# tancredeguillou/diner

Measured on AMD Instinct MI355X. Metric: rendered rays/sec (512x512, 4 src views, 128 samples/ray), higher is better.
Workload: dtype f32 (GEMM operands split into fp16 hi+lo, 3 fp16 MFMAs per product, fp32 accumulate)

## Files before the change

### diner_amd/_lib.py

```python
from __future__ import annotations

import ctypes as C
from pathlib import Path

import torch

LIB_PATH = Path(__file__).resolve().parent / "lib" / "libdiner_hip.so"
_FP = C.c_void_p

N_BLOCKS, COMBINE = 5, 3
ABI_VERSION = 3
PRECISIONS = {"fp32": 0, "f16x3": 1}
ROUNDINGS = {"save_image": 0, "video": 1}
BG_RULES = {"none": 0, "below_half": 1, "below_one": 2}
RESIZE_MODES = {"bilinear_aa": 1, "bilinear": 2, "bicubic_u8": 3}
ACT_NONE, ACT_RELU, ACT_SOFTPLUS = 0, 1, 2


class DinerScene(C.Structure):
    _fields_ = [("SB", C.c_int32), ("NV", C.c_int32), ("H", C.c_int32), ("W", C.c_int32),
                ("h", C.c_int32), ("w", C.c_int32), ("C", C.c_int32), ("num_freqs", C.c_int32),
                ("image_w", C.c_float), ("image_h", C.c_float), ("feature_padding", C.c_float),
                ("freq_factor", C.c_float),
                ("poses", _FP), ("focal", _FP), ("c", _FP), ("maps", _FP), ("latent", _FP), ("linz_maps", _FP)]
# ... 67 lines not shown
    "diner_gen_rays": (C.c_int, [_P, _P, _P, _P, _I32, _I32, _I32, _P, _P]),
    "diner_gen_rays_backward_workspace_floats": (_I64, [_I32, _I32, _I32]),
    "diner_gen_rays_backward": (C.c_int, [_P, _P, _P, _I32, _I32, _I32, _P, _P, _P, _P, _P, _P]),
    "diner_depth2normal": (C.c_int, [_P, _P, _I32, _I32, _I32, _P, _P]),
    "diner_pack_maps": (C.c_int, [_P, _P, _P, _I64, _I32, _I32, _P, _P]),
    "diner_pack_maps_from_depth": (C.c_int, [_P, _P, _P, _I64, _I32, _I32, _P, _P]),
    "diner_pack_latent": (C.c_int, [_P, _I64, _I32, _I32, _I32, _P, _P]),
    "diner_mlp_packed_floats": (_I64, []),
    "diner_pack_mlp": (C.c_int, [C.POINTER(DinerMlpRaw), _P, _P]),
    "diner_pack_linz_maps": (C.c_int, [_P, _I64, _I32, _I32, _P, _P, _P]),
    "diner_sample_coarse": (C.c_int, [_P, _I64, _I32, _P, _U64, _P, _P]),
    "diner_sample_depthguided": (C.c_int, [C.POINTER(DinerScene), _P, _I64, C.POINTER(DinerSamplerCfg),
                                           _P, _P, _P, _P, _U64, _P, _P, _P, _P]),
    "diner_fill_up_uniform_samples": (C.c_int, [_P, _P, _I64, _I32, _P, _U64, _P, _P]),
    "diner_render_points_scratch_floats": (_I64, [_I64, _I32, _I32]),
    "diner_render_points": (C.c_int, [C.POINTER(DinerScene), _P, _P, _P, _I64, _I32, _I32, _P, _P, _P]),
    "diner_composite": (C.c_int, [_P, _P, _P, _I64, _I32, _I32, _P, _P, _P, _P, _P]),
    "diner_decode_depth_u16": (C.c_int, [_P, _P, _P, _I64, _I32, _I32, _I32, C.c_float, C.c_float, C.c_float, C.c_float, C.c_float,
                                         _P, _P, _P, _P]),
    "diner_train_gemm": (C.c_int, [_P, _P, _P, _P, _P, _I64, _I32, _I32, _I64, _I64, _I64, _I64, _I64, _I64, _I32, _I32, _I32, _I32, _I64,
                                   _I32, _P, _P, _I32, _I32, _P]),
    "diner_train_amax": (C.c_int, [_P, _I64, _P, _P]),
    "diner_train_colsum_amax": (C.c_int, [_P, _I64, _I32, _I64, _P, _P, _P]),
    "diner_train_split_panel": (C.c_int, [_P, _I32, _I64, _I32, _I32, _P, _P, _P]),
    "diner_train_pack_core": (C.c_int, [_P, _I64, _I32, _I32, _P, _P]),
    "diner_train_gemm_core": (C.c_int, [_P, _I64, _P, _P, _P, _I64, _P, _I64, _P, _I64, _I64, _I32, _P, _I32, _I32, _P, _P, _P]),
    "diner_train_gemm_panel": (C.c_int, [_P, _I64, _P, _P, _P, _P, _I64, _P, _I64, _P, _I64, _I64, _I32, _I32, _P, _I32, _I32, _P]),
    "diner_train_colsum": (C.c_int, [_P, _I64, _I32, _I64, _P, _P]),
    "diner_train_point_inputs": (C.c_int, [C.POINTER(DinerScene), _P, _I32, _P, _P, _I64, _I32, _I32, _P, _P, _P, _P]),
    "diner_train_bilinear_scatter": (C.c_int, [_P, _P, _I64, _I32, _I32, _I32, _I32, _I32, _P, _P]),
# ... 146 lines not shown
        if not LIB_PATH.exists():
            raise ImportError(
                f"{LIB_PATH} is missing: the MI355X render path has no CPU or PyTorch fallback. "
                "Build it with `make -C diner_amd/csrc` (hipcc --offload-arch=gfx950).")
        l = C.CDLL(str(LIB_PATH))
        for name, (res, args) in SYMBOLS.items():
            fn = getattr(l, name)
            fn.restype, fn.argtypes = res, args
        if l.diner_version() != ABI_VERSION:
            raise ImportError(f"{LIB_PATH} has ABI version {l.diner_version()}, this binding needs {ABI_VERSION}: rebuild it "
                              "(`make -C diner_amd/csrc`)")
        _lib = l
    return _lib


def check(rc: int, what: str) -> None:
    if rc != 0:
        msg = lib().diner_last_error().decode(errors="replace")
        if rc == -1:
            raise ValueError(f"{what}: {msg}")
        if rc == -3:
            raise NotImplementedError(f"{what}: {msg}")
        raise DinerHipError(f"{what}: {msg} (rc={rc})")
```

### diner_amd/csrc/api.hip

```cpp
#include <stdarg.h>
#include <stdio.h>

#include <atomic>

#include "common.hpp"

namespace diner {

static thread_local char g_err[512] = "";

void set_error(const char *fmt, ...)
{
    va_list ap;
    va_start(ap, fmt);
    vsnprintf(g_err, sizeof(g_err), fmt, ap);
    va_end(ap);
}

int check_launch(const char *what)
{
    const hipError_t e = hipGetLastError();
    if (e != hipSuccess) {
        set_error("%s: %s", what, hipGetErrorString(e));
        return DINER_E_LAUNCH;
// ... 77 lines not shown
int launch_decode_depth(const unsigned short *, const unsigned short *, const unsigned short *, int64_t, int, int, int, float, float, float,
                        float, float, float *, float *, float *, hipStream_t);
int launch_linz_maps(const float *, int64_t, const float *, float *, hipStream_t);
int launch_linz_maps_ring(const float *, int64_t, int, int, const float *, float *, hipStream_t);
int launch_sampler(const DinerScene &, const float *, const DinerTargetCam *, float *, int64_t, const DinerSamplerCfg &, const float *,
                   const float *, const float *, const float *, uint64_t, float *, float *, float *, hipStream_t);
int launch_sampler_points(const DinerScene &, const float *, const float *, const float *, int64_t, const DinerSamplerCfg &, const float *,
                          const float *, uint64_t, float *, float *, float *, hipStream_t);
int launch_sample_coarse(const float *, int64_t, int, const float *, uint64_t, float *, hipStream_t);
int launch_fill_up(const float *, const float *, int64_t, int, const float *, uint64_t, float *, hipStream_t);
int launch_points_mlp(const DinerScene &, const DinerLatentIndex &, const float *, const float *, const float *, int64_t, int, float *, hipStream_t);
int64_t mlp_f16_packed_floats();
int launch_pack_mlp_f16(const DinerMlpRaw &, float *, hipStream_t);
int launch_points_mlp_f16(const DinerScene &, const DinerLatentIndex &, const float *, const float *, const float *, int64_t, int, float *, float *, hipStream_t);
int64_t points_mlp_f16_scratch_floats(int64_t SB, int NV);
namespace gen {
int check_shape(const DinerMlpShape &);
int64_t packed_floats(const DinerMlpShape &);
int launch_pack_mlp(const DinerMlpShape &, const DinerMlpGenRaw &, float *, hipStream_t);
int launch_points_mlp(const DinerScene &, const DinerLatentIndex &, const DinerMlpShape &, const float *, const float *, const float *, int64_t, int, float *, hipStream_t,
                      int bicubic_pad = -1);
int launch_points_mlp_lz(const DinerScene &, const DinerLatentIndex &, const DinerMlpShape &, const float *, const float *, const float *, int64_t, int, float *,
                         hipStream_t, int bicubic_pad, const float *lzmaps);
int64_t linz_maps_floats(const DinerMlpShape &, int64_t texels);
int launch_linz_maps(const DinerMlpShape &, const float *, int64_t, const float *, float *, hipStream_t);
int launch_points_mlp_novel(const DinerScene &, const DinerLatentIndex &, const DinerNovelGen &, const DinerMlpShape &, const float *, const float *,
                            const float *, const float *, int64_t, float *, hipStream_t);
int launch_points_mlp_novel_pe(const DinerScene &, const DinerLatentIndex &, const DinerNovelGen &, const DinerNovelPe &, const DinerMlpShape &,
                               const float *, const float *, const float *, const float *, const float *, int64_t, float *, hipStream_t);
int launch_novel_pe_map(const float *, int64_t, int, const float *, float *, hipStream_t);
// ... 233 lines not shown
    if (N < 0 || h <= 0 || w <= 0) return bad("linz_maps_floats: bad size");
    const int r = (index && index->padding == DINER_INDEX_PAD_ZEROS) ? 1 : 0;
    return 3 * N * (int64_t)(h + 2 * r) * (w + 2 * r) * DINER_D_LATENT;
}

int diner_pack_linz_maps_ix(const float *latent_packed, int64_t N, int32_t h, int32_t w, const float *mlp_packed,
                            const DinerLatentIndex *index, float *out, void *stream)
{
    int rc;
    if ((rc = check_index(index, "pack_linz_maps_ix"))) return rc;
    if (!index || index->padding != DINER_INDEX_PAD_ZEROS) return diner_pack_linz_maps(latent_packed, N, h, w, mlp_packed, out, stream);
    if (!latent_packed || !mlp_packed || !out) return bad("pack_linz_maps_ix: NULL pointer");
    if (N < 0 || h <= 0 || w <= 0) return bad("pack_linz_maps_ix: bad size");
    return launch_linz_maps_ring(latent_packed, N, h, w, mlp_packed, out, (hipStream_t)stream);
}

int64_t diner_render_points_scratch_floats(int64_t SB, int32_t NV, int32_t precision)
{
    return precision == DINER_PRECISION_F16X3 ? points_mlp_f16_scratch_floats(SB, NV) : 0;
}

int diner_render_points(const DinerScene *scene, const float *mlp_packed, const float *rays, const float *z,
                        int64_t NR, int32_t K, int32_t precision, float *scratch, float *rgbsigma_out, void *stream)
{
    return diner_render_points_ix(scene, nullptr, mlp_packed, rays, z, NR, K, precision, scratch, rgbsigma_out, stream);
}

int diner_render_points_ix(const DinerScene *scene, const DinerLatentIndex *index, const float *mlp_packed, const float *rays,
                           const float *z, int64_t NR, int32_t K, int32_t precision, float *scratch, float *rgbsigma_out, void *stream)
{
// ... 827 lines not shown
```

### diner_amd/csrc/common.hpp

```cpp
#pragma once
#include <hip/hip_runtime.h>
#include <stdint.h>

#include "../../include/diner_hip.h"

#define DINER_WAVE 64
#define DINER_SIGMA_PAD 100

namespace diner {

void set_error(const char *fmt, ...);
int check_launch(const char *what);

int device_cus();
enum LdsSlot { LDS_SLOT_F16_LINZ = 0, LDS_SLOT_F16_LATENT = 2, LDS_SLOT_F16_TRACE = 4, LDS_SLOT_TRAIN_CORE0 = 6, LDS_SLOT_DW512 = 10,
               LDS_SLOT_F16_GIX = 12, LDS_SLOT_COUNT = 16 };
int ensure_dynamic_lds(const void *kernel, int bytes, int slot);

struct View {
    float r[9];
    float t[3];
    float fx, fy, cx, cy;
};

__device__ __forceinline__ View load_view(const DinerScene &s, int sb, int v)
{
    View o;
    const float *P = s.poses + ((int64_t)sb * s.NV + v) * 16;
#pragma unroll
    for (int i = 0; i < 3; ++i) {
        o.r[i * 3 + 0] = P[i * 4 + 0];
// ... 315 lines not shown
```

### diner_amd/csrc/points_mlp_f16.hip

```cpp
#include <stdio.h>
#include <stdlib.h>

#include <type_traits>

#include "common.hpp"

namespace diner {

typedef float f32x16 __attribute__((ext_vector_type(16)));
typedef float f32x4 __attribute__((ext_vector_type(4)));
typedef _Float16 h8 __attribute__((ext_vector_type(8)));
typedef _Float16 h4 __attribute__((ext_vector_type(4)));
typedef unsigned u32x2 __attribute__((ext_vector_type(2)));

namespace f16x3 {

#include "f16_core16.inc"
#ifdef DINER_F16_DIAG
#include "f16_core16_trace.inc"
#endif
static_assert(F16_SHAPE == 16, "this kernel's glue is written for the 16x16x32 accumulator layout");

constexpr int TILE_P = 64;
constexpr int NWAVES = 8;
// ... 33 lines not shown
    int nkb, in_dim;
    if (i < OFF_LIN_Z) { w = raw.lin_in_w; rel = i; nkb = NKB_IN; in_dim = DINER_D_IN; }
    else if (i < OFF_FC0) { const int b = (int)((i - OFF_LIN_Z) / W_FULL); w = raw.lin_z_w[b]; rel = (i - OFF_LIN_Z) % W_FULL; nkb = NKB_FULL; in_dim = HID; }
    else if (i < OFF_FC1) { const int b = (int)((i - OFF_FC0) / W_FULL); w = raw.fc0_w[b]; rel = (i - OFF_FC0) % W_FULL; nkb = NKB_FULL; in_dim = HID; }
    else { const int b = (int)((i - OFF_FC1) / W_FULL); w = raw.fc1_w[b]; rel = (i - OFF_FC1) % W_FULL; nkb = NKB_FULL; in_dim = HID; }
    const int j = (int)(rel & 7), lane = (int)((rel >> 3) & 63), part = (int)((rel >> 9) & 1), tf2 = (int)((rel >> 10) & 1), hs = (int)((rel >> 11) & 1);
    const int64_t blk = rel >> 12;
    const int nks = nkb / 2, ks = (int)(blk % nks), wv = (int)(blk / nks);
    const int n = wv * 64 + 16 * (2 * hs + tf2) + (lane & 15), k = ks * 32 + 8 * (lane >> 4) + j;
    const float v = k < in_dim ? w[(int64_t)n * in_dim + k] : 0.0f;
    const _Float16 hi = (_Float16)v;
    outw[i] = part == 0 ? hi : (_Float16)(v - (float)hi);
}
#endif

template <int I, int N, class F> __device__ __forceinline__ void sfor(F &&f)
{
    if constexpr (I < N) {
        f(std::integral_constant<int, I>{});
        sfor<I + 1, N>(f);
    }
}
template <int N> __device__ __forceinline__ float acc_read()
{
    float v;
    asm volatile("v_mov_b32 %0, v%c1" : "=v"(v) : "n"(N));
    return v;
}
template <int N> __device__ __forceinline__ void acc_write(float v)
{
// ... 4 lines not shown
    asm volatile("v_add_f32 v%c0, v%c0, %1" ::"n"(N), "v"(v));
}
template <int N> __device__ __forceinline__ void acc_load4(const float *p)
{
    asm volatile("global_load_dwordx4 v[%c0:%c1], %2, off" ::"n"(N), "n"(N + 3), "v"(p) : "memory");
}
typedef __attribute__((address_space(1))) f32x4 g_f32x4;
typedef __attribute__((address_space(1))) unsigned g_u32;
typedef __attribute__((address_space(3))) volatile unsigned lds_vu32;
__device__ __forceinline__ f32x4 gload4(const float *p) { return *(const g_f32x4 *)p; }
__device__ __forceinline__ void gstore4(float *p, f32x4 v)
{
    asm volatile("global_store_dwordx4 %0, %1, off\n\ts_nop 3" ::"v"(p), "v"(v) : "memory");
}
template <int BASE, int TF, int TP, int I> constexpr int areg() { return BASE + 4 * (4 * TF + TP) + I; }

__device__ __forceinline__ void split(float s, _Float16 &hi, _Float16 &lo)
{
    hi = (_Float16)s;
    lo = (_Float16)(s - (float)hi);
}

constexpr int IMG_BYTES = 128 * 1024;
struct Tap {
    unsigned o00, o01, o10, o11;
    float nw, ne, sw, se;
};
constexpr int LDS_TAPS = IMG_BYTES;
constexpr int LDS_BIAS = LDS_TAPS + TILE_P * 32;
constexpr int LDS_FLAG = LDS_BIAS + BIAS_FLOATS * 4;
// ... 93 lines not shown
                     "v_pk_add_f32 v[%c[a2]:%c[a3]], v[%c[a2]:%c[a3]], v[%c[d2]:%c[d3]]\n\t"
                     "global_store_dwordx4 %[px], v[%c[x00]:%c[x03]], off\n\t"
                     "global_store_dwordx4 %[pn], v[%c[a0]:%c[a3]], off\n\t"
                     "s_nop 3"
                     ::[a0] "n"(n0), [a1] "n"(n0 + 1), [a2] "n"(n0 + 2), [a3] "n"(n0 + 3), [d0] "n"(n3), [d1] "n"(n3 + 1), [d2] "n"(n3 + 2), [d3] "n"(n3 + 3),
                       [x00] "n"(x0), [x01] "n"(x0 + 1), [x02] "n"(x0 + 2), [x03] "n"(x0 + 3), [x30] "n"(x3), [x31] "n"(x3 + 1), [x32] "n"(x3 + 2), [x33] "n"(x3 + 3),
                       [px] "v"(px), [pn] "v"(pn)
                     : "memory");
}

constexpr int SLAB_FLOATS = TILE_P * HID;
constexpr int PACE_EVERY = 4;
constexpr int TRACE_EVENTS = 512;
constexpr int SYNC_WORDS = 256;

template <bool LINZ, bool TRACE, bool VIT, class... IX>
__global__ __launch_bounds__(NWAVES * 64) __attribute__((amdgpu_num_vgpr(F16_VGPR_CAP / 2)))    void points_mlp_f16_kernel(
    DinerScene s, const float *__restrict__ Wp, const float *__restrict__ rays, const float *__restrict__ zsamp, int64_t NR, int K,
    int64_t tiles, float *__restrict__ scratch, float *__restrict__ rgbsigma, unsigned long long *__restrict__ dbg, IX... ix)
{
    constexpr bool GIX = sizeof...(IX) == 2;
    const int ixv[] = {ix..., 0, 0};
    const int ix_interp = GIX ? ixv[0] : 0, ix_padding = GIX ? ixv[1] : 0;
    int ev = 0;
    bool trace_on = false;
#define EV(ID)                                                                                   \
    if (TRACE && trace_on) {                                                                     \
        const unsigned long long t_ = __builtin_amdgcn_s_memtime();                              \
        if (lane == 0 && ev < TRACE_EVENTS) dbg[(wave * TRACE_EVENTS + ev) * 2] = t_, dbg[(wave * TRACE_EVENTS + ev) * 2 + 1] = ID; \
        ++ev;                                                                                    \
    }
#ifndef DINER_F16_DIAG
#define LAYER(FN, ...) FN(__VA_ARGS__)
#else
#define LAYER(FN, ...)                                                                           \
    do {                                                                                         \
        if constexpr (TRACE) {                                                                   \
// ... 30 lines not shown
        asm volatile("" : "+s"(b));
        (void)tn;
        return b + (uint64_t)(off_halfs * 2);
    };
    auto win = [&](int tn) -> uint64_t {
        uint64_t b = wbase_in;
        asm volatile("" : "+s"(b));
        (void)tn;
        return b;
    };
    const int ring = (GIX && LINZ && ix_padding == DINER_INDEX_PAD_ZEROS) ? 1 : 0;
    const int mw = s.w + 2 * ring, mh = s.h + 2 * ring;
    auto gmap = [&](int b, int v) -> uint64_t {
        uint64_t g = (uint64_t)(uintptr_t)s.linz_maps;
        asm volatile("" : "+s"(g));
        return g + (uint64_t)((((int64_t)b * s.SB + sb) * s.NV + v) * mh * mw) * (HID * 4);
    };
    GatherRegs greg;
    {
        const unsigned pl = lane >> 4, quad = lane & 15, stage = (unsigned)(uintptr_t)img + wave * 16384;
        greg.tbase = (unsigned)(uintptr_t)taps + pl * 32;
        greg.qb = wave * 256 + quad * 16;
#pragma unroll
        for (int k = 0; k < 4; ++k) greg.sw[k] = stage + pl * 256 + (((quad ^ pl) ^ (4 * k)) << 4);
        greg.rb = stage + c16 * 256;
        greg.hp = q ^ c16;
    }
    const unsigned loff = lane * 16;
    const unsigned ab0 = (unsigned)(uintptr_t)img + q * 2048 + c16 * 16;
    float *slab0 = scratch + SYNC_WORDS + ((int64_t)blockIdx.y * gridDim.x + blockIdx.x) * (int64_t)(2 * SLAB_FLOATS) + lane * 4;
    float *xs = slab0 + wave * (64 * 64);
// ... 29 lines not shown
                __hip_atomic_fetch_add(pace, 1u, __ATOMIC_RELAXED, __HIP_MEMORY_SCOPE_AGENT);
                const unsigned int want = (unsigned int)(round / PACE_EVERY + 1) * group;
                int spin = 0;
                for (; spin < 4000; ++spin) {
                    if (__hip_atomic_load(pace, __ATOMIC_RELAXED, __HIP_MEMORY_SCOPE_AGENT) >= want) break;
                    __builtin_amdgcn_s_sleep(8);
                }
                pace_flag[0] = spin < 4000;
            }
            __builtin_amdgcn_s_waitcnt(0xC07F);
            __builtin_amdgcn_s_barrier();
            pace_on = pace_flag[0] != 0;
        }
        trace_on = TRACE && blockIdx.x == 0 && blockIdx.y == 0 && round == 2;
        EV(1)
        int64_t p = tile * TILE_P + lane;
        if (p > P - 1) p = P - 1;
        const int64_t ray = p / K;
        const float *rp = rays + ((int64_t)sb * NR + ray) * 8;
        const float zz = zsamp[(int64_t)sb * P + p];
        const float dwx0 = rp[3], dwy0 = rp[4], dwz0 = rp[5];
        const float wx0 = rp[0] + zz * dwx0, wy0 = rp[1] + zz * dwy0, wz0 = rp[2] + zz * dwz0;
        float dwx = dwx0, dwy = dwy0, dwz = dwz0, wx = wx0, wy = wy0, wz = wz0;
        const int NG = VIT ? s.NV / 4 : 1;
        const int nph = VIT ? 4 * NG : s.NV;

#pragma unroll 1
        for (int ph = 0; ph < nph; ++ph) {
            const int v = VIT ? 4 * (ph % NG) : ph;
            const int sub = VIT ? ph / NG : 0;
            {
                const int tpv = VIT ? lane >> 4 : 0;
                if (VIT) {
                    const int src = 16 * sub + (lane & 15);
                    wx = __shfl(wx0, src, 64); wy = __shfl(wy0, src, 64); wz = __shfl(wz0, src, 64);
                    dwx = __shfl(dwx0, src, 64); dwy = __shfl(dwy0, src, 64); dwz = __shfl(dwz0, src, 64);
                }
                const View vw = load_view(s, sb, v + tpv);
                float px, py, pz, u, w;
                project(vw, s.image_w, s.image_h, wx, wy, wz, px, py, pz, u, w);
                float dcx, dcy, dcz;
                rotate(vw, dwx, dwy, dwz, dcx, dcy, dcz);
                const int row8 = (wave + 3) & 7;
                float delta = 0.0f;
                if ((unsigned)(row8 - 5) < 2u) {
                    const float4 *tex = (const float4 *)s.maps + ((int64_t)sb * s.NV + v + tpv) * s.H * s.W * 2;
                    const int ddx = safe_idx(__builtin_rintf(clipf(unnorm(u, (float)s.W / 2.0f), (float)(s.W - 1))), s.W);
                    const int ddy = safe_idx(__builtin_rintf(clipf(unnorm(w, (float)s.H / 2.0f), (float)(s.H - 1))), s.H);
                    delta = tex[((int64_t)ddy * s.W + ddx) * 2].w - pz;
                }
                const float half_pi = 1.5707963267948966f;
#pragma unroll 1
                for (int e8 = 0; e8 < 8; ++e8) {
                    const int e = row8 * 8 + e8;
                    _Float16 *cell = (_Float16 *)(img + row8 * 2048 + lane * 16);
                    const bool pe3 = e >= 3 && e < 39, pe1 = e >= 43 && e < 55;
                    const int j = pe3 ? (e - 3) / 3 : e - 43, i = pe3 ? (e - 3) % 3 : e < 3 ? e : e - 39;
                    const float comp = i == 0 ? px : i == 1 ? py : pz, dcomp = i == 0 ? dcx : i == 1 ? dcy : dcz;
                    const float src = pe1 ? delta : comp;
                    float sn = 0.0f;
                    if (pe3 || pe1) sn = pe_sin(__builtin_fmaf(src, s.freq_factor * (float)(1 << ((j >> 1) & 7)), (j & 1) ? half_pi : 0.0f));
// ... 20 lines not shown
            }
            if (LINZ) {
                EV(10) LAYER(layer_x_in0, win(0), win(1), wfull(OFF_FC0, 0), wfull(OFF_FC0, 1), loff, ab0, (++sy.lay, sy)); EV(11)
            } else {
                acc_bias<X, false>(bias, wave, q);
                EV(10) LAYER(layer_x_in, win(0), win(1), wfull(OFF_LIN_Z, 0), wfull(OFF_LIN_Z, 1), loff, ab0, (++sy.lay, sy)); EV(11)
            }

#pragma unroll 1
            for (int b = 0; b < DINER_COMBINE_LAYER; ++b) {
                if (LINZ) {
                    if (b == 0) gather_finish<false>(gmap(b, v), greg);
                    else gather_finish<true>(gmap(b, v), greg);
                    EV(60)
                } else {
                    const f32x4 *lat = (const f32x4 *)s.latent + ((int64_t)sb * s.NV + v) * s.h * s.w * (HID / 4);
                    const int half = wave >> 2, ur = half * 32 + c;
#pragma unroll 1
                    for (int r0 = 0; r0 < 16; r0 += 2) {
                        const int row = (wave & 3) * 16 + r0 + h;
                        const Tap t = taps[row];
                        h8 vh, vl;
#pragma unroll
                        for (int hf = 0; hf < 2; ++hf) {
                            const int q = 2 * ur + hf;
                            const f32x4 a = lat[t.o00 + q], bq = lat[t.o01 + q], cq = lat[t.o10 + q], d = lat[t.o11 + q];
#pragma unroll
                            for (int i = 0; i < 4; ++i) {
                                const float o = __builtin_fmaf(d[i], t.se, __builtin_fmaf(cq[i], t.sw, __builtin_fmaf(bq[i], t.ne, a[i] * t.nw)));
                                _Float16 hi, lo;
                                split(o * ACT_SCALE, hi, lo);
// ... 17 lines not shown
                    const bool to_in = b == DINER_COMBINE_LAYER - 1 && ph < nph - 1;
                    const uint64_t n0 = to_in ? win(0) : wfull(OFF_FC1 + b * W_FULL, 0), n1 = to_in ? win(1) : wfull(OFF_FC1 + b * W_FULL, 1);
                    EV(20) LAYER(layer_net_full, wfull(OFF_FC0 + b * W_FULL, 0), wfull(OFF_FC0 + b * W_FULL, 1), n0, n1, loff, ab0, (++sy.lay, sy)); EV(21)
                }
                if (b < DINER_COMBINE_LAYER - 1) {
                    store_relu<NET>(img, wave, c16, q);
                    EV(51)
                    if (!LINZ) acc_bias<X, true>(bias + 512 * (9 + b), wave, q);
                    EV(52)
                    const int64_t nxt = LINZ ? OFF_FC0 + (b + 1) * W_FULL : OFF_LIN_Z + (b + 1) * W_FULL;
                    if (LINZ) gather_issue(gmap(b + 1, v), greg);
                    EV(53)
                    EV(30) LAYER(layer_x_full, wfull(OFF_FC1 + b * W_FULL, 0), wfull(OFF_FC1 + b * W_FULL, 1), wfull(nxt, 0), wfull(nxt, 1), loff, ab0, (++sy.lay, sy)); EV(31)
                }
            }
            if (!VIT && v < s.NV - 1) {
                float *sl = xs;
                asm volatile("" : "+v"(sl));
                sfor<0, 4>([&](auto B4) {
                    f32x4 ax[4], an[4];
                    if (v > 0)
                        sfor<0, 4>([&](auto Q) { constexpr int Gq = 4 * B4 + Q; ax[Q.value] = gload4(sl + Gq * 256); an[Q.value] = gload4(sl + SLAB_FLOATS + Gq * 256); });
                    sfor<0, 4>([&](auto Q) {
                        constexpr int Gq = 4 * B4 + Q;
                        f32x4 vx, vn;
                        sfor<0, 4>([&](auto J) {
                            vx[J.value] = acc_read<X + 4 * Gq + J>();
                            const float n = acc_read<NET + 4 * Gq + J>();
                            vn[J.value] = n < 0.0f ? 0.0f : n;
                        });
                        if (v > 0) { vx = ax[Q.value] + vx; vn = an[Q.value] + vn; }
                        gstore4(sl + Gq * 256, vx);
                        gstore4(sl + SLAB_FLOATS + Gq * 256, vn);
                    });
                });
            }
            if (VIT) {
                const bool last = ph == nph - 1;
                float *sl = slab0 + sub * (2 * 8192) + wave * 1024;
                asm volatile("" : "+v"(sl));
                const bool part = v > 0;
                if (part) {
                    f32x4 px = gload4(sl), pn = gload4(sl + 8192);
                    sfor<0, 4>([&](auto TF) {
                        constexpr int tf = TF.value;
                        f32x4 qx = px, qn = pn;
                        if (tf < 3) { px = gload4(sl + (tf + 1) * 256); pn = gload4(sl + 8192 + (tf + 1) * 256); }
                        f32x4 sx, sn;
                        sfor<0, 4>([&](auto J) {
                            constexpr int j = J.value;
                            float ax = acc_read<areg<X, tf, 0, j>()>();
                            float n0 = acc_read<areg<NET, tf, 0, j>()>();
                            float an = n0 < 0.0f ? 0.0f : n0;
                            ax = qx[j] + ax; an = qn[j] + an;
                            sfor<1, 4>([&](auto TP) {
                                ax = ax + acc_read<areg<X, tf, TP.value, j>()>();
                                const float n = acc_read<areg<NET, tf, TP.value, j>()>();
// ... 5 lines not shown
                        if (last) {
                            sfor<0, 4>([&](auto J) { acc_write<areg<X, tf, 3, J.value>()>(sx[J.value]); acc_write<areg<NET, tf, 3, J.value>()>(sn[J.value]); });
                        } else {
                            gstore4(sl + tf * 256, sx);
                            gstore4(sl + 8192 + tf * 256, sn);
                        }
                    });
                }
                else if (last) sfor<0, 4>([&](auto TF) { vit_sum_tile<TF.value, true>(nullptr, nullptr); });
                else sfor<0, 4>([&](auto TF) { vit_sum_tile<TF.value, false>(sl + TF.value * 256, sl + 8192 + TF.value * 256); });
            }
        }
#pragma unroll 1
        for (int b = DINER_COMBINE_LAYER - 1; b < DINER_N_BLOCKS; ++b) {
            if (b == DINER_COMBINE_LAYER - 1) {
                const float nv = (float)s.NV;
                const bool pow2 = (s.NV & (s.NV - 1)) == 0;
                const float rnv = 1.0f / nv;
                const float *b1 = bias + 512 * (9 + DINER_COMBINE_LAYER - 1);
                const float *sl = xs;
                asm volatile("" : "+v"(sl));
                if (VIT) {
                    const float *sp = slab0 + wave * 1024;
                    asm volatile("" : "+v"(sp));
                    sfor<0, 12>([&](auto I) {
                        constexpr int sb3 = I.value / 4, tf = I.value % 4;
                        acc_load4<areg<X, tf, sb3, 0>()>(sp + sb3 * (2 * 8192) + tf * 256);
                        acc_load4<areg<NET, tf, sb3, 0>()>(sp + sb3 * (2 * 8192) + 8192 + tf * 256);
                    });
                    asm volatile("s_waitcnt vmcnt(0)" ::: "memory");
                }
                auto mean_step = [&](auto POW2) {
                sfor<0, 4>([&](auto B4) {
                    f32x4 ax[4], an[4];
                    if (!VIT && s.NV > 1)
                        sfor<0, 4>([&](auto Q) { constexpr int Gq = 4 * B4 + Q; ax[Q.value] = gload4(sl + Gq * 256); an[Q.value] = gload4(sl + SLAB_FLOATS + Gq * 256); });
                    sfor<0, 4>([&](auto Q) {
                        constexpr int Gq = 4 * B4 + Q, tf = Gq / 4, tp = Gq % 4;
                        f32x4 sx, sn;
                        sfor<0, 4>([&](auto J) {
                            sx[J.value] = acc_read<X + 4 * Gq + J>();
                            const float n = acc_read<NET + 4 * Gq + J>();
                            sn[J.value] = n < 0.0f ? 0.0f : n;
                        });
                        if (!VIT && s.NV > 1) { sx = ax[Q.value] + sx; sn = an[Q.value] + sn; }
                        const f32x4 bb = *(const f32x4 *)(b1 + wave * 64 + tf * 16 + 4 * q);
                        h4 vh, vl;
                        sfor<0, 4>([&](auto J) {
                            acc_write<X + 4 * Gq + J>((POW2.value ? sx[J.value] * rnv : sx[J.value] / nv) + bb[J.value]);
                            _Float16 hi, lo;
                            split(POW2.value ? sn[J.value] * rnv : sn[J.value] / nv, hi, lo);
                            vh[J.value] = hi;
                            vl[J.value] = lo;
                        });
                        char *pc = img + (wave * 8 + tf * 2 + (q >> 1)) * 2048 + (tp * 16 + c16) * 16 + 8 * (q & 1);
                        *(h4 *)pc = vh;
                        *(h4 *)(pc + 1024) = vl;
                    });
                });
                };
                if (pow2) mean_step(std::true_type{});
                else mean_step(std::false_type{});
            } else {
                store_relu<X>(img, wave, c16, q);
                acc_bias<NET, false>(bias + 512 * (4 + b), wave, q);
                EV(20) LAYER(layer_net_full, wfull(OFF_FC0 + b * W_FULL, 0), wfull(OFF_FC0 + b * W_FULL, 1), wfull(OFF_FC1 + b * W_FULL, 0),
                               wfull(OFF_FC1 + b * W_FULL, 1), loff, ab0, (++sy.lay, sy)); EV(21)
                store_relu<NET>(img, wave, c16, q);
                acc_bias<X, true>(bias + 512 * (9 + b), wave, q);
            }
            const bool last = b == DINER_N_BLOCKS - 1;
            const uint64_t n0 = last ? win(0) : wfull(OFF_FC0 + (b + 1) * W_FULL, 0), n1 = last ? win(1) : wfull(OFF_FC0 + (b + 1) * W_FULL, 1);
            EV(30) LAYER(layer_x_full, wfull(OFF_FC1 + b * W_FULL, 0), wfull(OFF_FC1 + b * W_FULL, 1), n0, n1, loff, ab0, (++sy.lay, sy)); EV(31)
        }
        {
            float part[4][4] = {};
            sfor<0, 4>([&](auto TF) {
                constexpr int tf = TF.value;
                const int f = wave * 64 + tf * 16 + 4 * q;
                f32x4 wo[4];
#pragma unroll
                for (int o = 0; o < 4; ++o) wo[o] = *(const f32x4 *)(Wout + o * 512 + f);
                sfor<0, 16>([&](auto PJ) {
                    constexpr int tp = PJ / 4, j = PJ % 4;
                    const float xv = acc_read<areg<X, tf, tp, j>()>();
                    const float a = xv < 0.0f ? 0.0f : xv;
#pragma unroll
                    for (int o = 0; o < 4; ++o) part[tp][o] = __builtin_fmaf(a, wo[o][j], part[tp][o]);
                });
            });
            f32x4 mine;
#pragma unroll
            for (int o = 0; o < 4; ++o) {
                float sel = 0.0f;
#pragma unroll
                for (int tp = 0; tp < 4; ++tp) {
                    float t = part[tp][o];
// ... 11 lines not shown
                flow_signal(sy.ctr + 16, sy.one);
                if (wave >= 4) head_ok = flow_wait(sy.ctr + 16, 8 * tiles_done);
            } else {
                __builtin_amdgcn_s_waitcnt(0xC07F);
                __builtin_amdgcn_s_barrier();
            }
            EV(41)
            if (wave >= 4) {
                const int t = tid - 256, pt = t >> 2, o = t & 3;
                float sum = 0.0f;
#pragma unroll
                for (int w8 = 0; w8 < 8; ++w8) sum += *(const float *)(img + head_slot(w8) + pt * 16 + o * 4);
                if (F16_FLOW && *(lds_vu32 *)(lds + LDS_CTR + F16_POISON_OFF) != 0) head_ok = false;
                if (!head_ok) sum = __builtin_nanf("");
                const float val = (sum + bias[14 * 512 + o]) * (1.0f / ACT_SCALE);
                const int64_t pp = tile * TILE_P + pt;
                if (pp < P) rgbsigma[((int64_t)sb * P + pp) * 4 + o] = o < 3 ? 1.0f / (1.0f + expf(-val)) : (val < 0.0f ? 0.0f : val);
            }
            EV(42)
        }
    }
#undef EV
#undef LAYER
    if (!F16_FLOW && wave < 4) __builtin_amdgcn_s_barrier();
    asm volatile("s_waitcnt vmcnt(0)" ::: "memory");
}

}

#ifndef DINER_F16_KERNEL_ONLY
int64_t mlp_f16_packed_floats() { return f16x3::PACKED_FLOATS; }

int launch_pack_mlp_f16(const DinerMlpRaw &raw, float *out, hipStream_t st)
{
    using namespace f16x3;
    hipLaunchKernelGGL(pack_kernel, dim3((unsigned)((W_HALFS + 255) / 256)), dim3(256), 0, st, raw, (_Float16 *)out,
                       out + W_HALFS / 2);
    return check_launch("f16x3::pack_kernel");
}

const void *points_mlp_f16_gix_kernel(bool linz, bool vit);

static bool getenv_no_vit()
{
    static const bool off = getenv("DINER_F16_NO_VIT") != nullptr;
    return off;
}

static int f16_grid_limit() { return device_cus(); }

int64_t points_mlp_f16_scratch_floats(int64_t SB, int NV)
{
    return f16x3::SYNC_WORDS + (NV > 1 ? (int64_t)f16_grid_limit() * SB * 2 * f16x3::SLAB_FLOATS : 0);
}

int launch_points_mlp_f16(const DinerScene &s, const DinerLatentIndex &ix, const float *mlp_packed, const float *rays, const float *z,
                          int64_t NR, int K, float *scratch, float *rgbsigma, hipStream_t st)
{
    using namespace f16x3;
    const int64_t P = NR * (int64_t)K;
    if (P == 0 || s.SB == 0) return DINER_OK;
    if (s.C != DINER_D_LATENT) { set_error("render_points: latent channels C=%d unsupported (need %d)", s.C, DINER_D_LATENT); return DINER_E_UNSUPPORTED; }
    if (s.num_freqs != 6) { set_error("render_points: num_freqs=%d unsupported (need 6)", s.num_freqs); return DINER_E_UNSUPPORTED; }
    if (!scratch) { set_error("render_points(f16x3): scratch is NULL"); return DINER_E_INVALID; }
    if (hipMemsetAsync(scratch, 0, SYNC_WORDS * sizeof(float), st) != hipSuccess) return check_launch("memset(pacing counters)");
    const int64_t tiles = (P + TILE_P - 1) / TILE_P;
    const int64_t grid = tiles < f16_grid_limit() ? tiles : f16_grid_limit();
    const bool vit = s.NV % 4 == 0 && !getenv_no_vit();
    const bool gix = ix.interp != DINER_INDEX_BILINEAR || ix.padding != DINER_INDEX_PAD_BORDER;
    const void *fn = gix ? points_mlp_f16_gix_kernel(s.linz_maps != nullptr, vit)
                         : (s.linz_maps ? (vit ? (const void *)points_mlp_f16_kernel<true, false, true> : (const void *)points_mlp_f16_kernel<true, false, false>)
                                        : (vit ? (const void *)points_mlp_f16_kernel<false, false, true> : (const void *)points_mlp_f16_kernel<false, false, false>));
    if (const int rc = ensure_dynamic_lds(fn, LDS_BYTES, (s.linz_maps ? LDS_SLOT_F16_LINZ : LDS_SLOT_F16_LATENT) + (vit ? 1 : 0) + (gix ? LDS_SLOT_F16_GIX : 0)))
        return rc;
    const int ii = ix.interp, ip = ix.padding;
#ifdef DINER_F16_DIAG
    static const bool trace = getenv("DINER_F16_TRACE") != nullptr;
    if (trace && s.linz_maps && gix) {
        set_error("render_points(f16x3): DINER_F16_TRACE serves the bilinear / border lookup only (index interp=%d padding=%d)", ii, ip);
        return DINER_E_UNSUPPORTED;
    }
    if (trace && s.linz_maps) {
        static unsigned long long *dbg = nullptr;
        const size_t nb = NWAVES * TRACE_EVENTS * 2 * sizeof(unsigned long long);
        if (!dbg && hipMalloc(&dbg, nb) != hipSuccess) return DINER_E_LAUNCH;
        (void)hipMemsetAsync(dbg, 0, nb, st);
        const void *tfn = vit ? (const void *)points_mlp_f16_kernel<true, true, true> : (const void *)points_mlp_f16_kernel<true, true, false>;
        if (const int rc = ensure_dynamic_lds(tfn, LDS_BYTES, LDS_SLOT_F16_TRACE + (vit ? 1 : 0))) return rc;
        void *targs[] = {(void *)&s, (void *)&mlp_packed, (void *)&rays, (void *)&z, (void *)&NR, (void *)&K, (void *)&tiles, (void *)&scratch, (void *)&rgbsigma, (void *)&dbg};
        if (hipLaunchKernel(tfn, dim3((unsigned)grid, (unsigned)s.SB), dim3(NWAVES * 64), targs, LDS_BYTES, st) != hipSuccess) return check_launch("points_mlp_f16_kernel<trace>(launch)");
        static unsigned long long h[NWAVES * TRACE_EVENTS * 2];
        (void)hipStreamSynchronize(st);
        (void)hipMemcpy(h, dbg, nb, hipMemcpyDeviceToHost);
        for (int w = 0; w < NWAVES; ++w) {
            fprintf(stderr, "[f16 trace] wave%d:", w);
            for (int e = 0; e < TRACE_EVENTS && h[(w * TRACE_EVENTS + e) * 2 + 1]; ++e)
                fprintf(stderr, " %llu:%llu", h[(w * TRACE_EVENTS + e) * 2 + 1], h[(w * TRACE_EVENTS + e) * 2] - h[0]);
            fprintf(stderr, "\n");
        }
        return check_launch("points_mlp_f16_kernel<trace>");
    }
#endif
    unsigned long long *nodbg = nullptr;
    void *kargs[] = {(void *)&s, (void *)&mlp_packed, (void *)&rays, (void *)&z, (void *)&NR, (void *)&K, (void *)&tiles, (void *)&scratch, (void *)&rgbsigma, (void *)&nodbg, (void *)&ii, (void *)&ip};
    if (hipLaunchKernel(fn, dim3((unsigned)grid, (unsigned)s.SB), dim3(NWAVES * 64), kargs, LDS_BYTES, st) != hipSuccess)
        return check_launch("points_mlp_f16_kernel(launch)");
    return check_launch("points_mlp_f16_kernel");
}
#endif

}
```

### include/diner_hip.h

```cpp
#ifndef DINER_HIP_H
#define DINER_HIP_H

#include <stdint.h>

#ifdef __cplusplus
extern "C" {
#endif

#define DINER_OK 0
#define DINER_E_INVALID (-1)
#define DINER_E_LAUNCH (-2)
#define DINER_E_UNSUPPORTED (-3)

#define DINER_D_LATENT 512
#define DINER_D_HIDDEN 512
#define DINER_D_IN 55
#define DINER_N_BLOCKS 5
#define DINER_COMBINE_LAYER 3
#define DINER_MAP_TEXEL 8

#define DINER_PRECISION_FP32 0
#define DINER_PRECISION_F16X3 1

typedef struct DinerScene {
// ... 111 lines not shown
int diner_sample_coarse(const float *rays, int64_t N, int32_t NC, const float *u_coarse, uint64_t seed,
                        float *z_out, void *stream);
int diner_fill_up_uniform_samples(const float *rays, const float *z_in, int64_t N, int32_t K,
                                  const float *u_fill, uint64_t seed, float *z_out, void *stream);

int diner_sample_depthguided(const DinerScene *scene, const float *rays, int64_t NR,
                             const DinerSamplerCfg *cfg, const float *u_coarse,
                             const float *n_gauss, const float *u_fill, const float *z_cand,
                             uint64_t seed, float *z_out, float *z_dg_out, float *lik_out,
                             void *stream);

int64_t diner_render_points_scratch_floats(int64_t SB, int32_t NV, int32_t precision);
int diner_render_points(const DinerScene *scene, const float *mlp_packed, const float *rays,
                        const float *z, int64_t NR, int32_t K, int32_t precision, float *scratch,
                        float *rgbsigma_out, void *stream);
int diner_render_points_ix(const DinerScene *scene, const DinerLatentIndex *index, const float *mlp_packed, const float *rays,
                           const float *z, int64_t NR, int32_t K, int32_t precision, float *scratch, float *rgbsigma_out,
                           void *stream);

#define DINER_STATUS_NONFINITE 1u
int diner_composite(const float *rays, const float *z, const float *rgbsigma, int64_t N, int32_t K,
                    int32_t white_bkgd, float *rgb_out, float *depth_out, float *weights_out,
                    uint32_t *status, void *stream);

int64_t diner_render_workspace_floats(int64_t SB, int64_t NR, int32_t K, int32_t NV, int32_t precision);
int diner_render(const DinerScene *scene, const float *mlp_packed, const float *rays, int64_t NR,
                 const DinerSamplerCfg *cfg, int32_t white_bkgd, int32_t precision, const float *u_coarse,
                 const float *n_gauss, const float *u_fill, uint64_t seed, float *workspace,
                 float *rgb_out, float *depth_out, float *weights_out, uint32_t *status, void *stream);
int diner_render_ix(const DinerScene *scene, const DinerLatentIndex *index, const float *mlp_packed, const float *rays, int64_t NR,
// ... 295 lines not shown
```

Measured before the change: 265,200.

## Add compile-time four-view specialization of f16 points MLP kernel with 32-bit indexing

Adds a template specialization of the f16x3 points MLP kernel where the view count is a compile-time constant (4). With a fixed count the compiler can fold view-dependent address arithmetic, pick the power-of-two mean path statically and skip the partial-sum global reload in the views-in-tile reduction. It also switches to 32-bit index arithmetic when sizes allow and loads output weights through scalar registers. The change adds a separate kernel instantiation and LDS slot, plus a debug query that reports which variant last ran. It only applies when NV==4 with linz maps and the default index mode.

```diff
diff --git a/diner_amd/_lib.py b/diner_amd/_lib.py
--- a/diner_amd/_lib.py
+++ b/diner_amd/_lib.py
@@ -105,6 +105,7 @@
                                            _P, _P, _P, _P, _U64, _P, _P, _P, _P]),
     "diner_fill_up_uniform_samples": (C.c_int, [_P, _P, _I64, _I32, _P, _U64, _P, _P]),
     "diner_render_points_scratch_floats": (_I64, [_I64, _I32, _I32]),
+    "diner_points_mlp_f16_last_kernel": (_I32, []),
     "diner_render_points": (C.c_int, [C.POINTER(DinerScene), _P, _P, _P, _I64, _I32, _I32, _P, _P, _P]),
     "diner_composite": (C.c_int, [_P, _P, _P, _I64, _I32, _I32, _P, _P, _P, _P, _P]),
     "diner_decode_depth_u16": (C.c_int, [_P, _P, _P, _I64, _I32, _I32, _I32, C.c_float, C.c_float, C.c_float, C.c_float, C.c_float,
@@ -281,6 +282,14 @@
     return _lib
 
 
+F16_KERNEL_BITS = {"linz": 1, "vit": 2, "gix": 4, "nv4": 8, "idx32": 16}
+
+
+def f16_last_kernel():
+    code = int(lib().diner_points_mlp_f16_last_kernel())
+    return None if code < 0 else frozenset(k for k, b in F16_KERNEL_BITS.items() if code & b)
+
+
 def check(rc: int, what: str) -> None:
     if rc != 0:
         msg = lib().diner_last_error().decode(errors="replace")
diff --git a/diner_amd/csrc/api.hip b/diner_amd/csrc/api.hip
--- a/diner_amd/csrc/api.hip
+++ b/diner_amd/csrc/api.hip
@@ -115,6 +115,7 @@
 int launch_pack_mlp_f16(const DinerMlpRaw &, float *, hipStream_t);
 int launch_points_mlp_f16(const DinerScene &, const DinerLatentIndex &, const float *, const float *, const float *, int64_t, int, float *, float *, hipStream_t);
 int64_t points_mlp_f16_scratch_floats(int64_t SB, int NV);
+int points_mlp_f16_last_kernel();
 namespace gen {
 int check_shape(const DinerMlpShape &);
 int64_t packed_floats(const DinerMlpShape &);
@@ -378,6 +379,8 @@
     if (N < 0 || h <= 0 || w <= 0) return bad("pack_linz_maps_ix: bad size");
     return launch_linz_maps_ring(latent_packed, N, h, w, mlp_packed, out, (hipStream_t)stream);
 }
+
+int32_t diner_points_mlp_f16_last_kernel(void) { return points_mlp_f16_last_kernel(); }
 
 int64_t diner_render_points_scratch_floats(int64_t SB, int32_t NV, int32_t precision)
 {
diff --git a/diner_amd/csrc/common.hpp b/diner_amd/csrc/common.hpp
--- a/diner_amd/csrc/common.hpp
+++ b/diner_amd/csrc/common.hpp
@@ -14,7 +14,7 @@
 
 int device_cus();
 enum LdsSlot { LDS_SLOT_F16_LINZ = 0, LDS_SLOT_F16_LATENT = 2, LDS_SLOT_F16_TRACE = 4, LDS_SLOT_TRAIN_CORE0 = 6, LDS_SLOT_DW512 = 10,
-               LDS_SLOT_F16_GIX = 12, LDS_SLOT_COUNT = 16 };
+               LDS_SLOT_F16_GIX = 12, LDS_SLOT_F16_NV4 = 16, LDS_SLOT_COUNT = 18 };
 int ensure_dynamic_lds(const void *kernel, int bytes, int slot);
 
 struct View {
diff --git a/diner_amd/csrc/points_mlp_f16.hip b/diner_amd/csrc/points_mlp_f16.hip
--- a/diner_amd/csrc/points_mlp_f16.hip
+++ b/diner_amd/csrc/points_mlp_f16.hip
@@ -1,6 +1,7 @@
 #include <stdio.h>
 #include <stdlib.h>
 
+#include <atomic>
 #include <type_traits>
 
 #include "common.hpp"
@@ -71,6 +72,12 @@
 }
 #endif
 
+template <int N> struct NvViews { int idx32; };
+template <class... IX> struct nvc_of { static constexpr int value = 0; };
+template <int N> struct nvc_of<NvViews<N>> { static constexpr int value = N; };
+__device__ __forceinline__ int ix_word(int v) { return v; }
+template <int N> __device__ __forceinline__ int ix_word(NvViews<N> v) { return v.idx32; }
+
 template <int I, int N, class F> __device__ __forceinline__ void sfor(F &&f)
 {
     if constexpr (I < N) {
@@ -105,6 +112,22 @@
     asm volatile("global_store_dwordx4 %0, %1, off\n\ts_nop 3" ::"v"(p), "v"(v) : "memory");
 }
 template <int BASE, int TF, int TP, int I> constexpr int areg() { return BASE + 4 * (4 * TF + TP) + I; }
+
+__device__ __forceinline__ View load_view_at(const DinerScene &s, int64_t i)
+{
+    View o;
+    const float *P = s.poses + i * 16;
+#pragma unroll
+    for (int r = 0; r < 3; ++r) {
+        o.r[r * 3 + 0] = P[r * 4 + 0];
+        o.r[r * 3 + 1] = P[r * 4 + 1];
+        o.r[r * 3 + 2] = P[r * 4 + 2];
+        o.t[r] = P[r * 4 + 3];
+    }
+    const float *f = s.focal + i * 2, *c = s.c + i * 2;
+    o.fx = f[0]; o.fy = f[1]; o.cx = c[0]; o.cy = c[1];
+    return o;
+}
 
 __device__ __forceinline__ void split(float s, _Float16 &hi, _Float16 &lo)
 {
@@ -228,13 +251,17 @@
 constexpr int TRACE_EVENTS = 512;
 constexpr int SYNC_WORDS = 256;
 
+#define DINER_SNV (NVC ? NVC : s.NV)
 template <bool LINZ, bool TRACE, bool VIT, class... IX>
 __global__ __launch_bounds__(NWAVES * 64) __attribute__((amdgpu_num_vgpr(F16_VGPR_CAP / 2)))    void points_mlp_f16_kernel(
     DinerScene s, const float *__restrict__ Wp, const float *__restrict__ rays, const float *__restrict__ zsamp, int64_t NR, int K,
     int64_t tiles, float *__restrict__ scratch, float *__restrict__ rgbsigma, unsigned long long *__restrict__ dbg, IX... ix)
 {
+    constexpr int NVC = nvc_of<IX...>::value;
+    static_assert(NVC == 0 || (VIT && NVC % 4 == 0), "a compile-time view count serves the views-in-tile form");
     constexpr bool GIX = sizeof...(IX) == 2;
-    const int ixv[] = {ix..., 0, 0};
+    const int ixv[] = {ix_word(ix)..., 0, 0};
+    const bool idx32 = NVC != 0 && ixv[0] != 0;
     const int ix_interp = GIX ? ixv[0] : 0, ix_padding = GIX ? ixv[1] : 0;
     int ev = 0;
     bool trace_on = false;
@@ -295,7 +322,7 @@
     auto gmap = [&](int b, int v) -> uint64_t {
         uint64_t g = (uint64_t)(uintptr_t)s.linz_maps;
         asm volatile("" : "+s"(g));
-        return g + (uint64_t)((((int64_t)b * s.SB + sb) * s.NV + v) * mh * mw) * (HID * 4);
+        return g + (uint64_t)((((int64_t)b * s.SB + sb) * DINER_SNV + v) * mh * mw) * (HID * 4);
     };
     GatherRegs greg;
     {
@@ -355,16 +382,27 @@
         }
         trace_on = TRACE && blockIdx.x == 0 && blockIdx.y == 0 && round == 2;
         EV(1)
-        int64_t p = tile * TILE_P + lane;
-        if (p > P - 1) p = P - 1;
-        const int64_t ray = p / K;
-        const float *rp = rays + ((int64_t)sb * NR + ray) * 8;
-        const float zz = zsamp[(int64_t)sb * P + p];
+        const float *rp;
+        float zz;
+        if (NVC != 0 && idx32) {
+            const unsigned P32 = (unsigned)P;
+            unsigned p = (unsigned)tile * TILE_P + lane;
+            if (p > P32 - 1) p = P32 - 1;
+            const unsigned ray = p / (unsigned)K;
+            rp = rays + (uint64_t)((unsigned)sb * (unsigned)NR + ray) * 8;
+            zz = zsamp[(unsigned)sb * P32 + p];
+        } else {
+            int64_t p = tile * TILE_P + lane;
+            if (p > P - 1) p = P - 1;
+            const int64_t ray = p / K;
+            rp = rays + ((int64_t)sb * NR + ray) * 8;
+            zz = zsamp[(int64_t)sb * P + p];
+        }
         const float dwx0 = rp[3], dwy0 = rp[4], dwz0 = rp[5];
         const float wx0 = rp[0] + zz * dwx0, wy0 = rp[1] + zz * dwy0, wz0 = rp[2] + zz * dwz0;
         float dwx = dwx0, dwy = dwy0, dwz = dwz0, wx = wx0, wy = wy0, wz = wz0;
-        const int NG = VIT ? s.NV / 4 : 1;
-        const int nph = VIT ? 4 * NG : s.NV;
+        const int NG = VIT ? DINER_SNV / 4 : 1;
+        const int nph = VIT ? 4 * NG : DINER_SNV;
 
 #pragma unroll 1
         for (int ph = 0; ph < nph; ++ph) {
@@ -377,7 +415,7 @@
                     wx = __shfl(wx0, src, 64); wy = __shfl(wy0, src, 64); wz = __shfl(wz0, src, 64);
                     dwx = __shfl(dwx0, src, 64); dwy = __shfl(dwy0, src, 64); dwz = __shfl(dwz0, src, 64);
                 }
-                const View vw = load_view(s, sb, v + tpv);
+                const View vw = NVC ? load_view_at(s, (int64_t)sb * NVC + tpv) : load_view(s, sb, v + tpv);
                 float px, py, pz, u, w;
                 project(vw, s.image_w, s.image_h, wx, wy, wz, px, py, pz, u, w);
                 float dcx, dcy, dcz;
@@ -385,7 +423,7 @@
                 const int row8 = (wave + 3) & 7;
                 float delta = 0.0f;
                 if ((unsigned)(row8 - 5) < 2u) {
-                    const float4 *tex = (const float4 *)s.maps + ((int64_t)sb * s.NV + v + tpv) * s.H * s.W * 2;
+                    const float4 *tex = (const float4 *)s.maps + ((int64_t)sb * DINER_SNV + v + tpv) * s.H * s.W * 2;
                     const int ddx = safe_idx(__builtin_rintf(clipf(unnorm(u, (float)s.W / 2.0f), (float)(s.W - 1))), s.W);
                     const int ddy = safe_idx(__builtin_rintf(clipf(unnorm(w, (float)s.H / 2.0f), (float)(s.H - 1))), s.H);
                     delta = tex[((int64_t)ddy * s.W + ddx) * 2].w - pz;
@@ -436,7 +474,7 @@
                     else gather_finish<true>(gmap(b, v), greg);
                     EV(60)
                 } else {
-                    const f32x4 *lat = (const f32x4 *)s.latent + ((int64_t)sb * s.NV + v) * s.h * s.w * (HID / 4);
+                    const f32x4 *lat = (const f32x4 *)s.latent + ((int64_t)sb * DINER_SNV + v) * s.h * s.w * (HID / 4);
                     const int half = wave >> 2, ur = half * 32 + c;
 #pragma unroll 1
                     for (int r0 = 0; r0 < 16; r0 += 2) {
@@ -484,7 +522,7 @@
                     EV(30) LAYER(layer_x_full, wfull(OFF_FC1 + b * W_FULL, 0), wfull(OFF_FC1 + b * W_FULL, 1), wfull(nxt, 0), wfull(nxt, 1), loff, ab0, (++sy.lay, sy)); EV(31)
                 }
             }
-            if (!VIT && v < s.NV - 1) {
+            if (!VIT && v < DINER_SNV - 1) {
                 float *sl = xs;
                 asm volatile("" : "+v"(sl));
                 sfor<0, 4>([&](auto B4) {
@@ -510,7 +548,11 @@
                 float *sl = slab0 + sub * (2 * 8192) + wave * 1024;
                 asm volatile("" : "+v"(sl));
                 const bool part = v > 0;
-                if (part) {
+                if constexpr (NVC == 4) {
+                    if (last) sfor<0, 4>([&](auto TF) { vit_sum_tile<TF.value, true>(nullptr, nullptr); });
+                    else sfor<0, 4>([&](auto TF) { vit_sum_tile<TF.value, false>(sl + TF.value * 256, sl + 8192 + TF.value * 256); });
+                }
+                else if (part) {
                     f32x4 px = gload4(sl), pn = gload4(sl + 8192);
                     sfor<0, 4>([&](auto TF) {
                         constexpr int tf = TF.value;
@@ -546,8 +588,8 @@
 #pragma unroll 1
         for (int b = DINER_COMBINE_LAYER - 1; b < DINER_N_BLOCKS; ++b) {
             if (b == DINER_COMBINE_LAYER - 1) {
-                const float nv = (float)s.NV;
-                const bool pow2 = (s.NV & (s.NV - 1)) == 0;
+                const float nv = (float)DINER_SNV;
+                const bool pow2 = (DINER_SNV & (DINER_SNV - 1)) == 0;
                 const float rnv = 1.0f / nv;
                 const float *b1 = bias + 512 * (9 + DINER_COMBINE_LAYER - 1);
                 const float *sl = xs;
@@ -565,7 +607,7 @@
                 auto mean_step = [&](auto POW2) {
                 sfor<0, 4>([&](auto B4) {
                     f32x4 ax[4], an[4];
-                    if (!VIT && s.NV > 1)
+                    if (!VIT && DINER_SNV > 1)
                         sfor<0, 4>([&](auto Q) { constexpr int Gq = 4 * B4 + Q; ax[Q.value] = gload4(sl + Gq * 256); an[Q.value] = gload4(sl + SLAB_FLOATS + Gq * 256); });
                     sfor<0, 4>([&](auto Q) {
                         constexpr int Gq = 4 * B4 + Q, tf = Gq / 4, tp = Gq % 4;
@@ -575,7 +617,7 @@
                             const float n = acc_read<NET + 4 * Gq + J>();
                             sn[J.value] = n < 0.0f ? 0.0f : n;
                         });
-                        if (!VIT && s.NV > 1) { sx = ax[Q.value] + sx; sn = an[Q.value] + sn; }
+                        if (!VIT && DINER_SNV > 1) { sx = ax[Q.value] + sx; sn = an[Q.value] + sn; }
                         const f32x4 bb = *(const f32x4 *)(b1 + wave * 64 + tf * 16 + 4 * q);
                         h4 vh, vl;
                         sfor<0, 4>([&](auto J) {
@@ -591,7 +633,8 @@
                     });
                 });
                 };
-                if (pow2) mean_step(std::true_type{});
+                if constexpr (NVC != 0) mean_step(std::integral_constant<bool, (NVC & (NVC - 1)) == 0>{});
+                else if (pow2) mean_step(std::true_type{});
                 else mean_step(std::false_type{});
             } else {
                 store_relu<X>(img, wave, c16, q);
@@ -611,8 +654,15 @@
                 constexpr int tf = TF.value;
                 const int f = wave * 64 + tf * 16 + 4 * q;
                 f32x4 wo[4];
-#pragma unroll
-                for (int o = 0; o < 4; ++o) wo[o] = *(const f32x4 *)(Wout + o * 512 + f);
+                if constexpr (NVC != 0) {
+                    const float *wout = Wout;
+                    asm volatile("" : "+s"(wout));
+#pragma unroll
+                    for (int o = 0; o < 4; ++o) wo[o] = gload4(wout + o * 512 + f);
+                } else {
+#pragma unroll
+                    for (int o = 0; o < 4; ++o) wo[o] = *(const f32x4 *)(Wout + o * 512 + f);
+                }
                 sfor<0, 16>([&](auto PJ) {
                     constexpr int tp = PJ / 4, j = PJ % 4;
                     const float xv = acc_read<areg<X, tf, tp, j>()>();
@@ -654,8 +704,13 @@
                 if (F16_FLOW && *(lds_vu32 *)(lds + LDS_CTR + F16_POISON_OFF) != 0) head_ok = false;
                 if (!head_ok) sum = __builtin_nanf("");
                 const float val = (sum + bias[14 * 512 + o]) * (1.0f / ACT_SCALE);
-                const int64_t pp = tile * TILE_P + pt;
-                if (pp < P) rgbsigma[((int64_t)sb * P + pp) * 4 + o] = o < 3 ? 1.0f / (1.0f + expf(-val)) : (val < 0.0f ? 0.0f : val);
+                if (NVC != 0 && idx32) {
+                    const unsigned pp = (unsigned)tile * TILE_P + pt;
+                    if (pp < (unsigned)P) rgbsigma[(uint64_t)((unsigned)sb * (unsigned)P + pp) * 4 + o] = o < 3 ? 1.0f / (1.0f + expf(-val)) : (val < 0.0f ? 0.0f : val);
+                } else {
+                    const int64_t pp = tile * TILE_P + pt;
+                    if (pp < P) rgbsigma[((int64_t)sb * P + pp) * 4 + o] = o < 3 ? 1.0f / (1.0f + expf(-val)) : (val < 0.0f ? 0.0f : val);
+                }
             }
             EV(42)
         }
@@ -665,6 +720,7 @@
     if (!F16_FLOW && wave < 4) __builtin_amdgcn_s_barrier();
     asm volatile("s_waitcnt vmcnt(0)" ::: "memory");
 }
+#undef DINER_SNV
 
 }
 
@@ -686,6 +742,20 @@
     static const bool off = getenv("DINER_F16_NO_VIT") != nullptr;
     return off;
 }
+
+const void *points_mlp_f16_nv4_kernel();
+#ifdef DINER_F16_DIAG
+const void *points_mlp_f16_nv4_trace_kernel();
+#endif
+
+static bool getenv_no_nv4()
+{
+    static const bool off = getenv("DINER_F16_NO_NV4") != nullptr;
+    return off;
+}
+
+static std::atomic<int> g_last_kernel{-1};
+int points_mlp_f16_last_kernel() { return g_last_kernel.load(std::memory_order_relaxed); }
 
 static int f16_grid_limit() { return device_cus(); }
 
@@ -708,12 +778,16 @@
     const int64_t grid = tiles < f16_grid_limit() ? tiles : f16_grid_limit();
     const bool vit = s.NV % 4 == 0 && !getenv_no_vit();
     const bool gix = ix.interp != DINER_INDEX_BILINEAR || ix.padding != DINER_INDEX_PAD_BORDER;
-    const void *fn = gix ? points_mlp_f16_gix_kernel(s.linz_maps != nullptr, vit)
+    const bool nv4 = s.linz_maps && vit && !gix && s.NV == 4 && !getenv_no_nv4();
+    const bool idx32 = nv4 && (int64_t)s.SB * P < (int64_t(1) << 31) && getenv("DINER_F16_FORCE_IDX64") == nullptr;
+    const void *fn = nv4 ? points_mlp_f16_nv4_kernel()
+                   : gix ? points_mlp_f16_gix_kernel(s.linz_maps != nullptr, vit)
                          : (s.linz_maps ? (vit ? (const void *)points_mlp_f16_kernel<true, false, true> : (const void *)points_mlp_f16_kernel<true, false, false>)
                                         : (vit ? (const void *)points_mlp_f16_kernel<false, false, true> : (const void *)points_mlp_f16_kernel<false, false, false>));
-    if (const int rc = ensure_dynamic_lds(fn, LDS_BYTES, (s.linz_maps ? LDS_SLOT_F16_LINZ : LDS_SLOT_F16_LATENT) + (vit ? 1 : 0) + (gix ? LDS_SLOT_F16_GIX : 0)))
+    if (const int rc = ensure_dynamic_lds(fn, LDS_BYTES, nv4 ? LDS_SLOT_F16_NV4 : (s.linz_maps ? LDS_SLOT_F16_LINZ : LDS_SLOT_F16_LATENT) + (vit ? 1 : 0) + (gix ? LDS_SLOT_F16_GIX : 0)))
         return rc;
     const int ii = ix.interp, ip = ix.padding;
+    const NvViews<4> nvarg = {idx32 ? 1 : 0};
 #ifdef DINER_F16_DIAG
     static const bool trace = getenv("DINER_F16_TRACE") != nullptr;
     if (trace && s.linz_maps && gix) {
@@ -725,9 +799,10 @@
         const size_t nb = NWAVES * TRACE_EVENTS * 2 * sizeof(unsigned long long);
         if (!dbg && hipMalloc(&dbg, nb) != hipSuccess) return DINER_E_LAUNCH;
         (void)hipMemsetAsync(dbg, 0, nb, st);
-        const void *tfn = vit ? (const void *)points_mlp_f16_kernel<true, true, true> : (const void *)points_mlp_f16_kernel<true, true, false>;
-        if (const int rc = ensure_dynamic_lds(tfn, LDS_BYTES, LDS_SLOT_F16_TRACE + (vit ? 1 : 0))) return rc;
-        void *targs[] = {(void *)&s, (void *)&mlp_packed, (void *)&rays, (void *)&z, (void *)&NR, (void *)&K, (void *)&tiles, (void *)&scratch, (void *)&rgbsigma, (void *)&dbg};
+        const void *tfn = nv4 ? points_mlp_f16_nv4_trace_kernel()
+                              : vit ? (const void *)points_mlp_f16_kernel<true, true, true> : (const void *)points_mlp_f16_kernel<true, true, false>;
+        if (const int rc = ensure_dynamic_lds(tfn, LDS_BYTES, nv4 ? LDS_SLOT_F16_NV4 + 1 : LDS_SLOT_F16_TRACE + (vit ? 1 : 0))) return rc;
+        void *targs[] = {(void *)&s, (void *)&mlp_packed, (void *)&rays, (void *)&z, (void *)&NR, (void *)&K, (void *)&tiles, (void *)&scratch, (void *)&rgbsigma, (void *)&dbg, (void *)&nvarg};
         if (hipLaunchKernel(tfn, dim3((unsigned)grid, (unsigned)s.SB), dim3(NWAVES * 64), targs, LDS_BYTES, st) != hipSuccess) return check_launch("points_mlp_f16_kernel<trace>(launch)");
         static unsigned long long h[NWAVES * TRACE_EVENTS * 2];
         (void)hipStreamSynchronize(st);
@@ -743,6 +818,9 @@
 #endif
     unsigned long long *nodbg = nullptr;
     void *kargs[] = {(void *)&s, (void *)&mlp_packed, (void *)&rays, (void *)&z, (void *)&NR, (void *)&K, (void *)&tiles, (void *)&scratch, (void *)&rgbsigma, (void *)&nodbg, (void *)&ii, (void *)&ip};
+    if (nv4) kargs[10] = (void *)&nvarg;
+    g_last_kernel.store((s.linz_maps ? DINER_F16_KERNEL_LINZ : 0) | (vit ? DINER_F16_KERNEL_VIT : 0) | (gix ? DINER_F16_KERNEL_GIX : 0) |
+                        (nv4 ? DINER_F16_KERNEL_NV4 : 0) | (idx32 ? DINER_F16_KERNEL_IDX32 : 0), std::memory_order_relaxed);
     if (hipLaunchKernel(fn, dim3((unsigned)grid, (unsigned)s.SB), dim3(NWAVES * 64), kargs, LDS_BYTES, st) != hipSuccess)
         return check_launch("points_mlp_f16_kernel(launch)");
     return check_launch("points_mlp_f16_kernel");
diff --git a/diner_amd/csrc/points_mlp_f16_nv4.hip b/diner_amd/csrc/points_mlp_f16_nv4.hip
--- /dev/null
+++ b/diner_amd/csrc/points_mlp_f16_nv4.hip
@@ -0,0 +1,20 @@
+#define DINER_F16_KERNEL_ONLY
+#include "points_mlp_f16.hip"
+
+namespace diner {
+
+const void *points_mlp_f16_nv4_kernel()
+{
+    using namespace f16x3;
+    return (const void *)points_mlp_f16_kernel<true, false, true, NvViews<4>>;
+}
+
+#ifdef DINER_F16_DIAG
+const void *points_mlp_f16_nv4_trace_kernel()
+{
+    using namespace f16x3;
+    return (const void *)points_mlp_f16_kernel<true, true, true, NvViews<4>>;
+}
+#endif
+
+}
diff --git a/include/diner_hip.h b/include/diner_hip.h
--- a/include/diner_hip.h
+++ b/include/diner_hip.h
@@ -149,6 +149,12 @@
 int diner_render_points(const DinerScene *scene, const float *mlp_packed, const float *rays,
                         const float *z, int64_t NR, int32_t K, int32_t precision, float *scratch,
                         float *rgbsigma_out, void *stream);
+#define DINER_F16_KERNEL_LINZ 1
+#define DINER_F16_KERNEL_VIT 2
+#define DINER_F16_KERNEL_GIX 4
+#define DINER_F16_KERNEL_NV4 8
+#define DINER_F16_KERNEL_IDX32 16
+int32_t diner_points_mlp_f16_last_kernel(void);
 int diner_render_points_ix(const DinerScene *scene, const DinerLatentIndex *index, const float *mlp_packed, const float *rays,
                            const float *z, int64_t NR, int32_t K, int32_t precision, float *scratch, float *rgbsigma_out,
                            void *stream);
```

Result: no change. 267,100, median of 6 (+0.7%).
